# cics-nd/gptorch

Measured on AMD Instinct MI355X. Metric: GP log-marginal-likelihood evals/sec (Cholesky+solve) at NxD fp64, higher is better.
Workload: dtype f64; 1 GPU; C3: GPR+Matern52 N=32768 D=16 fp64 LML eval; N=32768, D=16, dy=1, kernel=Matern52, parallelism=1 GPU

## Files before the change

### gptorch_amd/_native.py

```python
import ctypes
import os

_HERE = os.path.dirname(os.path.abspath(__file__))
LIB_PATH = os.environ.get("GPN_LIB", os.path.join(_HERE, "lib", "libgpnative.so"))

c_void_p, c_int, c_int64, c_double = ctypes.c_void_p, ctypes.c_int, ctypes.c_int64, ctypes.c_double

SIGNATURES = {
    "gpn_version": (c_int, []),
    "gpn_arch": (ctypes.c_char_p, []),
    "gpn_last_hip_error": (ctypes.c_char_p, []),
    "gpn_factor_ld": (c_int64, [c_int64, c_int64]),
    "gpn_factor_rows": (c_int64, [c_int64, c_int64]),
    "gpn_winv_bytes": (c_int64, [c_int64]),
    "gpn_kernel_matrix": (c_int, [c_void_p, c_int, c_void_p, c_int64, c_void_p, c_int64, c_int,
                                  c_void_p, c_void_p, c_int, c_void_p, c_int, c_void_p, c_int64]),
    "gpn_pack_rhs": (c_int, [c_void_p, c_void_p, c_void_p, c_int64, c_int, c_void_p, c_int64]),
    "gpn_potrf_lower": (c_int, [c_void_p, c_void_p, c_int64, c_int64, c_int64, c_void_p, c_void_p]),
    "gpn_potrf_lower_panel": (c_int, [c_void_p, c_void_p, c_int64, c_int64, c_int64, c_void_p, c_void_p]),
    "gpn_potrf_lower_batched": (c_int, [c_void_p, c_void_p, c_int64, c_int64, c_int64, c_int64, c_void_p, c_int64, c_void_p, c_int]),
    "gpn_lml_reduce_batched": (c_int, [c_void_p, c_void_p, c_int64, c_int64, c_int64, c_int64, c_void_p, c_int]),
    "gpn_lml_forward_batched": (c_int, [c_void_p, c_int, c_int, c_void_p, c_int64, c_int64, c_int, c_void_p, c_int64, c_void_p, c_int64, c_int,
                                        c_void_p, c_void_p, c_int, c_void_p, c_void_p, c_int64, c_int64, c_void_p, c_int64, c_void_p, c_void_p]),
    "gpn_potrf_panel_width": (c_int64, [c_int64]),
    "gpn_potrf_panel_levels": (c_int, [c_int64, c_void_p]),
    "gpn_potrf_lower_persistent": (c_int, [c_void_p, c_void_p, c_int64, c_int64, c_int64, c_void_p, c_void_p]),
    "gpn_potrf_persistent_supported": (c_int, [c_int64, c_int64]),
    "gpn_potrf_persistent_plan": (c_int, [c_int64, c_int64, c_void_p, c_void_p, c_int64, c_void_p, c_int64]),
    "gpn_release_stream": (c_int, [c_void_p]),
    "gpn_trtri_diag": (c_int, [c_void_p, c_void_p, c_int64, c_int64, c_void_p, c_void_p]),
    "gpn_trsm_right_lt": (c_int, [c_void_p, c_void_p, c_int64, c_int64, c_void_p, c_void_p, c_int64, c_int64]),
    "gpn_lml_reduce": (c_int, [c_void_p, c_void_p, c_int64, c_int64, c_int64, c_void_p]),
    "gpn_gemm_nt": (c_int, [c_void_p, c_int64, c_int64, c_int64, c_double, c_void_p, c_int64,
                            c_void_p, c_int64, c_double, c_void_p, c_int64, c_int, c_int]),
    "gpn_gemm_nt_stair": (c_int, [c_void_p, c_int64, c_int64, c_int64, c_int64, c_double, c_void_p, c_int64,
                                  c_void_p, c_int64, c_double, c_void_p, c_int64, c_int64, c_int]),
    "gpn_gemm_nt_batched": (c_int, [c_void_p, c_int64, c_int64, c_int64, c_double, c_void_p, c_int64, c_int64,
                                    c_void_p, c_int64, c_int64, c_double, c_void_p, c_int64, c_int64, c_int, c_int, c_int]),
    "gpn_gemm_nt_batched_scaled": (c_int, [c_void_p, c_int64, c_int64, c_int64, c_void_p, c_void_p, c_int64, c_int64,
                                           c_void_p, c_int64, c_int64, c_double, c_void_p, c_int64, c_int64, c_int, c_int, c_int]),
    "gpn_kernel_matrix_batched": (c_int, [c_void_p, c_int, c_int, c_void_p, c_int64, c_int64, c_void_p, c_int64, c_int64, c_int,
                                          c_void_p, c_void_p, c_int, c_void_p, c_int, c_void_p, c_int64, c_int64]),
    "gpn_trsm_right_lt_batched": (c_int, [c_void_p, c_void_p, c_int64, c_int64, c_int64, c_void_p, c_int64,
                                          c_void_p, c_int64, c_int64, c_int64, c_int]),
    "gpn_trtri_upper_batched": (c_int, [c_void_p, c_void_p, c_int64, c_int64, c_int64, c_void_p, c_int64,
                                        c_void_p, c_int64, c_int64, c_void_p, c_int64, c_int64, c_int]),
    "gpn_kernel_grad_batched": (c_int, [c_void_p, c_int, c_int, c_void_p, c_int64, c_int64, c_void_p, c_int64, c_int64, c_int,
                                        c_void_p, c_void_p, c_int, c_void_p, c_int64, c_int64, c_void_p, c_void_p]),
    "gpn_kernel_grad_x2_batched": (c_int, [c_void_p, c_int, c_int, c_void_p, c_int64, c_int64, c_void_p, c_int64, c_int64, c_int,
                                           c_void_p, c_void_p, c_int, c_void_p, c_int64, c_int64, c_double, c_int, c_void_p, c_void_p]),
    "gpn_dot2d_batched": (c_int, [c_void_p, c_void_p, c_int64, c_int64, c_void_p, c_int64, c_int64, c_int64, c_int64, c_void_p, c_int]),
    "gpn_lml_forward_ragged": (c_int, [c_void_p, c_int, c_int, c_void_p, c_int64, c_int64, c_void_p, c_int, c_void_p, c_int64, c_int,
                                       c_void_p, c_void_p, c_int, c_void_p, c_void_p, c_int64, c_int64, c_void_p, c_int64, c_void_p, c_void_p]),
    "gpn_lml_backward_ragged": (c_int, [c_void_p, c_int, c_int, c_void_p, c_int64, c_int64, c_void_p, c_int, c_void_p, c_void_p, c_int,
                                        c_void_p, c_int64, c_int64, c_void_p, c_int64, c_int, c_void_p, c_void_p]),
    "gpn_trtri_upper": (c_int, [c_void_p, c_void_p, c_int64, c_int64, c_void_p, c_void_p, c_int64]),
    "gpn_trtri_upper_ws": (c_int, [c_void_p, c_void_p, c_int64, c_int64, c_void_p, c_void_p, c_int64, c_void_p, c_int64]),
    "gpn_grad_work_bytes": (c_int64, [c_int64, c_int64, c_int, c_int]),
    "gpn_lml_grad": (c_int, [c_void_p, c_int, c_void_p, c_int64, c_int, c_void_p, c_void_p, c_int,
                             c_void_p, c_int64, c_void_p, c_int64, c_int, c_void_p, c_void_p]),
    "gpn_kernel_grad": (c_int, [c_void_p, c_int, c_void_p, c_int64, c_void_p, c_int64, c_int, c_void_p, c_void_p,
                                c_int, c_void_p, c_int64, c_void_p, c_void_p]),
    "gpn_grad_x2_work_bytes": (c_int64, [c_int64, c_int64, c_int]),
    "gpn_kernel_grad_x2": (c_int, [c_void_p, c_int, c_void_p, c_int64, c_void_p, c_int64, c_int, c_void_p, c_void_p,
                                   c_int, c_void_p, c_int64, c_double, c_int, c_void_p, c_void_p]),
    "gpn_lml_forward": (c_int, [c_void_p, c_int, c_void_p, c_int64, c_int, c_void_p, c_void_p, c_int, c_void_p, c_void_p,
                                c_int, c_void_p, c_void_p, c_int64, c_void_p, c_void_p, c_void_p]),
    "gpn_lml_forward_saving": (c_int, [c_void_p, c_int, c_void_p, c_int64, c_int, c_void_p, c_void_p, c_int, c_void_p, c_void_p,
                                       c_int, c_void_p, c_void_p, c_int64, c_void_p, c_void_p, c_void_p, c_void_p]),
    "gpn_lml_refine_work_bytes": (c_int64, [c_int64, c_int]),
    "gpn_lml_refine": (c_int, [c_void_p, c_int, c_void_p, c_int64, c_int, c_void_p, c_void_p, c_int, c_void_p, c_void_p,
                               c_int, c_void_p, c_void_p, c_int64, c_void_p, c_void_p, c_void_p]),
    "gpn_lml_backward_work_bytes": (c_int64, [c_int64, c_int, c_int]),
    "gpn_lml_backward": (c_int, [c_void_p, c_int, c_void_p, c_int64, c_int, c_void_p, c_void_p, c_int,
                                 c_void_p, c_int64, c_void_p, c_int, c_void_p, c_void_p, c_void_p]),
    "gpn_lml_backward_batched_work_bytes": (c_int64, [c_int64, c_int, c_int, c_int]),
    "gpn_lml_backward_batched": (c_int, [c_void_p, c_int, c_int, c_void_p, c_int64, c_int64, c_int, c_void_p, c_void_p, c_int,
                                         c_void_p, c_int64, c_int64, c_void_p, c_int64, c_int, c_void_p, c_void_p, c_void_p]),
    "gpn_lml_kinv_layout": (c_int, [c_int64, c_int, ctypes.POINTER(c_int64)]),
    "gpn_lml_kinv_batched_work_bytes": (c_int64, [c_int64, c_int, c_int]),
    "gpn_lml_kinv_batched": (c_int, [c_void_p, c_int, c_int64, c_void_p, c_int64, c_int64, c_void_p, c_int64, c_int, c_void_p]),
    "gpn_lml_grad_batched": (c_int, [c_void_p, c_int, c_int, c_void_p, c_int64, c_int64, c_int, c_void_p, c_void_p, c_int,
                                     c_void_p, c_int64, c_int64, c_void_p, c_int64, c_int64, c_int, c_void_p, c_void_p]),
    "gpn_predict_work_bytes": (c_int64, [c_int64, c_int64, c_int]),
    "gpn_predict": (c_int, [c_void_p, c_int, c_void_p, c_int64, c_int, c_void_p, c_int64, c_void_p, c_void_p, c_void_p, c_int,
                            c_void_p, c_int64, c_void_p, c_int, c_int, c_void_p, c_void_p, c_void_p]),
    "gpn_block_inverse_bytes": (c_int64, [c_int64]),
    "gpn_block_inverse": (c_int, [c_void_p, c_void_p, c_int64, c_int64, c_void_p, c_void_p]),
    "gpn_trsm_right_lt_blocked": (c_int, [c_void_p, c_void_p, c_int64, c_int64, c_void_p, c_void_p, c_int64, c_int64, c_void_p, c_int64]),
    "gpn_predict_blocked": (c_int, [c_void_p, c_int, c_void_p, c_int64, c_int, c_void_p, c_int64, c_void_p, c_void_p, c_void_p, c_int,
                                    c_void_p, c_int64, c_void_p, c_void_p, c_int, c_int, c_void_p, c_void_p, c_void_p]),
    "gpn_transpose": (c_int, [c_void_p, c_void_p, c_int64, c_int64, c_int64, c_void_p, c_int64]),
    "gpn_copy_matrix": (c_int, [c_void_p, c_void_p, c_int64, c_int64, c_int64, c_void_p, c_int64, c_int]),
    "gpn_row_sumsq": (c_int, [c_void_p, c_void_p, c_int64, c_int64, c_int64, c_void_p]),
    "gpn_fill_zero": (c_int, [c_void_p, c_void_p, c_int64]),
    "gpn_gemv_t_work_bytes": (c_int64, [c_int64, c_int64, c_int]),
    "gpn_gemv_t_acc": (c_int, [c_void_p, c_void_p, c_int64, c_int64, c_int64, c_void_p, c_int64, c_int, c_void_p, c_int64, c_void_p]),
    "gpn_refine_tile_count": (c_int64, [c_int64]),
    "gpn_refine_resid_part_work_bytes": (c_int64, [c_int, c_int64]),
    "gpn_refine_resid_part": (c_int, [c_void_p, c_int, c_void_p, c_int64, c_int, c_void_p, c_void_p, c_int, c_void_p,
                                      c_void_p, c_int, c_int64, c_int64, c_void_p, c_void_p]),
    "gpn_svgp_marginals": (c_int, [c_void_p, c_void_p, c_int64, c_void_p, c_int64, c_int64, c_int64, c_void_p, c_int64, c_int,
                                   c_void_p, c_int64, c_void_p, c_void_p]),
    "gpn_svgp_backward_rows": (c_int, [c_void_p, c_void_p, c_int64, c_void_p, c_int64, c_int64, c_int64, c_void_p, c_int64, c_int,
                                       c_void_p, c_void_p, c_void_p, c_void_p, c_int64]),
    "gpn_refine_finish": (c_int, [c_void_p, c_void_p, c_void_p, c_void_p, c_void_p, c_int64, c_int, c_void_p]),
}
class ExprTerm(ctypes.Structure):
    _fields_ = [("type", c_int), ("kind", c_int), ("var_off", c_int), ("ls_off", c_int), ("nls", c_int), ("nvar", c_int)]


TERM_STATIONARY, TERM_LINEAR, TERM_CONSTANT, TERM_WHITE = 0, 1, 2, 3
EXPR_MAX_TERMS, EXPR_MAX_GROUPS = 16, 8
SIGNATURES.update({
    "gpn_lml_refine_dense": (c_int, [c_void_p, c_void_p, c_int64, c_double, c_int64, c_void_p, c_void_p, c_int, c_void_p, c_int64, c_void_p, c_void_p, c_void_p]),
    "gpn_lml_refine_expr": (c_int, [c_void_p, ctypes.POINTER(ExprTerm), c_int, ctypes.POINTER(c_int), c_int, c_void_p, c_void_p, c_int64, c_int,
                                    c_void_p, c_void_p, c_int, c_void_p, c_void_p, c_int64, c_void_p, c_void_p, c_void_p]),
    "gpn_refine_resid_part_expr": (c_int, [c_void_p, ctypes.POINTER(ExprTerm), c_int, ctypes.POINTER(c_int), c_int, c_void_p, c_void_p, c_int64, c_int,
                                           c_void_p, c_void_p, c_int, c_int64, c_int64, c_void_p, c_void_p]),
    "gpn_kernel_matrix_expr": (c_int, [c_void_p, ctypes.POINTER(ExprTerm), c_int, ctypes.POINTER(c_int), c_int, c_void_p, c_void_p,
                                       c_int64, c_void_p, c_int64, c_int, c_void_p, c_int, c_void_p, c_int64]),
    "gpn_kernel_expr_grad_work_bytes": (c_int64, [c_int64, c_int64, c_int, c_int]),
    "gpn_kernel_matrix_expr_batched": (c_int, [c_void_p, ctypes.POINTER(ExprTerm), c_int, ctypes.POINTER(c_int), c_int, c_int, c_void_p,
                                               c_int64, c_void_p, c_int64, c_int64, c_int, c_void_p, c_void_p, c_int64, c_int64]),
    "gpn_kernel_expr_grad_batched": (c_int, [c_void_p, ctypes.POINTER(ExprTerm), c_int, ctypes.POINTER(c_int), c_int, c_int, c_void_p,
                                             c_int64, c_int, c_void_p, c_int64, c_int64, c_int, c_void_p, c_int64, c_int64, c_void_p,
                                             c_int64, c_int64, c_int, c_int, c_void_p, c_void_p]),
    "gpn_kernel_expr_grad": (c_int, [c_void_p, ctypes.POINTER(ExprTerm), c_int, ctypes.POINTER(c_int), c_int, c_void_p, c_int,
                                     c_void_p, c_int64, c_void_p, c_int64, c_int, c_void_p, c_int64, c_void_p, c_int64, c_int, c_int,
                                     c_void_p, c_void_p]),
})

BCAST_FN = ctypes.CFUNCTYPE(c_int, c_void_p, c_int, c_void_p, c_int64, c_int, c_void_p)
ALLREDUCE_FN = ctypes.CFUNCTYPE(c_int, c_void_p, c_void_p, c_int64, c_void_p)


class DistComm(ctypes.Structure):
    _fields_ = [("ctx", c_void_p), ("bcast", BCAST_FN), ("allreduce", ALLREDUCE_FN), ("flags", c_int)]


SIGNATURES.update({
    "gpn_dist_work_bytes": (c_int64, [c_int, c_int, c_int, c_int64, c_int, c_int, c_int64]),
    "gpn_dist_lml_refine_work_bytes": (c_int64, [c_int, c_int, c_int, c_int64, c_int, c_int, c_int64]),
    "gpn_dist_grad_work_bytes": (c_int64, [c_int, c_int, c_int, c_int64, c_int, c_int, c_int64]),
    "gpn_dist_lml_grad": (c_int, [c_void_p, ctypes.POINTER(DistComm), c_int, c_int, c_int, c_int, c_void_p, c_int64, c_int,
                                  c_void_p, c_int, c_void_p, c_void_p, c_int, c_void_p, c_int64, c_void_p, c_int64, c_void_p,
                                  c_void_p, c_void_p]),
    "gpn_dist_layout": (c_int, [c_int, c_int, c_int, c_int, c_int64, c_int, c_int, c_int64, ctypes.POINTER(c_int64), c_int]),
    "gpn_dist_predict_work_bytes": (c_int64, [c_int, c_int, c_int, c_int64, c_int, c_int, c_int64, c_int64, c_int]),
    "gpn_dist_predict": (c_int, [c_void_p, ctypes.POINTER(DistComm), c_int, c_int, c_int, c_int, c_void_p, c_int64, c_int,
                                 c_void_p, c_int, c_void_p, c_int64, c_void_p, c_void_p, c_void_p, c_int, c_void_p, c_int64, c_int,
                                 c_void_p, c_int64, c_void_p, c_void_p, c_void_p]),
    "gpn_dist_lml_forward": (c_int, [c_void_p, ctypes.POINTER(DistComm), c_int, c_int, c_int, c_int, c_void_p, c_int64, c_int,
                                     c_void_p, c_int, c_void_p, c_void_p, c_int, c_void_p, c_int64, c_void_p, c_int64, c_void_p]),
    "gpn_dist_lml_refine": (c_int, [c_void_p, ctypes.POINTER(DistComm), c_int, c_int, c_int, c_int, c_void_p, c_int64, c_int,
                                    c_void_p, c_int, c_void_p, c_void_p, c_int, c_void_p, c_int64, c_void_p, c_void_p, c_int64, c_void_p]),
})
RCCL_LIB_PATH = os.environ.get("GPN_RCCL_LIB", os.path.join(os.path.dirname(LIB_PATH), "libgpnative_rccl.so"))
RCCL_SIGNATURES = {
    "gpn_rccl_comm_create": (ctypes.POINTER(DistComm), [c_void_p, c_void_p, c_void_p]),
    "gpn_rccl_comm_destroy": (None, [ctypes.POINTER(DistComm)]),
    "gpn_mesh_plan": (c_int64, [c_int, c_int, c_int, c_int64, c_int, c_int64, ctypes.POINTER(c_int64), c_int64]),
}
DIST_FORCE_COLLECTIVES, DIST_MESH_EXCHANGE = 1, 2
_rccl_lib = None


def rccl_lib():
    global _rccl_lib
    if _rccl_lib is None:
        if not os.path.exists(RCCL_LIB_PATH):
            raise NativeError("libgpnative_rccl.so not found at %s -- run gptorch_amd/csrc/build.sh" % RCCL_LIB_PATH)
        handle = ctypes.CDLL(RCCL_LIB_PATH)
        for name, (res, args) in RCCL_SIGNATURES.items():
            fn = getattr(handle, name)
            fn.restype, fn.argtypes = res, args
        _rccl_lib = handle
    return _rccl_lib


PROFILE_SIGNATURES = {
    "gpn_profile_enable": (c_int, [c_int]),
    "gpn_profile_collect": (c_int, [ctypes.POINTER(c_double)]),
    "gpn_profile_collect_classes": (c_int, [ctypes.POINTER(c_double), c_int]),
}
SIGNATURES.update(PROFILE_SIGNATURES)
DEBUG_SIGNATURES = {
    "gpn_debug_set_gemm_variant": (c_int, [c_int]),
    "gpn_debug_set_potrf_variant": (c_int, [c_int]),
    "gpn_debug_set_outer_width": (c_int, [c_int, c_int]),
    "gpn_debug_set_extra_rows": (c_int, [c_int]),
    "gpn_debug_set_thin_tiles": (c_int, [c_int]),
    "gpn_debug_masked_stream": (c_int, [ctypes.POINTER(ctypes.c_uint32), c_int, ctypes.POINTER(c_void_p)]),
    "gpn_debug_set_backsub_persistent": (c_int, [c_int]),
    "gpn_debug_set_persistent": (c_int, [c_int, c_int]),
    "gpn_debug_persistent_trace": (c_int, [c_void_p]),
}
DEBUG_LIB_PATH = os.path.join(_HERE, "lib", "libgpnative_dbg.so")

_lib = None
_product_lib = None
_debug_lib = None


class NativeError(RuntimeError):
    pass


def _load(path, extra):
    handle = ctypes.CDLL(path)
    for name, (res, args) in list(SIGNATURES.items()) + list(extra.items()):
        fn = getattr(handle, name)
        fn.restype, fn.argtypes = res, args
    return handle


def lib():
    global _lib, _product_lib
    if _lib is None:
        if not os.path.exists(LIB_PATH):
            raise NativeError(
                "libgpnative.so not found at %s -- build it with `python -c 'import __graft_entry__ as g; "
                "g.build()'` (or gptorch_amd/csrc/build.sh). gptorch_amd has no CPU fallback." % LIB_PATH)
        extra = DEBUG_SIGNATURES if os.path.basename(LIB_PATH).startswith("libgpnative_dbg") else {}
        _product_lib = _lib = _load(LIB_PATH, extra)
    return _lib


class debug_library:

    def __enter__(self):
        global _lib, _debug_lib
        lib()
        if _debug_lib is None:
            if not os.path.exists(DEBUG_LIB_PATH):
                raise NativeError("libgpnative_dbg.so not found at %s -- run gptorch_amd/csrc/build.sh" % DEBUG_LIB_PATH)
            _debug_lib = _load(DEBUG_LIB_PATH, DEBUG_SIGNATURES)
        _lib = _debug_lib
        return _debug_lib

    def __exit__(self, *exc):
        global _lib
        _debug_lib.gpn_debug_set_gemm_variant(0)
        _debug_lib.gpn_debug_set_potrf_variant(0)
        _lib = _product_lib
        return False


_debug_ctx = None


def debug_begin():
    global _debug_ctx
    if _debug_ctx is None:
        _debug_ctx = debug_library()
        return _debug_ctx.__enter__()
    return _debug_lib


def debug_end():
    global _debug_ctx
    if _debug_ctx is not None:
        _debug_ctx.__exit__(None, None, None)
        _debug_ctx = None


def check(status, what):
    if status != 0:
        detail = lib().gpn_last_hip_error().decode() if status == -100 else ""
        raise NativeError("%s failed with status %d %s" % (what, status, detail))
```

### gptorch_amd/csrc/gemm_f64.hip

```cpp
#include <algorithm>
#include <atomic>
#include <type_traits>
#include <cstdlib>
#include "gpn_common.h"
#include "gemm_tile.h"

namespace gpn {

template <int BM, int BN, int WM, int WN, bool DMA, int NS = 2, bool BLOW = false, bool PIPE = false>
__global__ __launch_bounds__(64 * (BM / WM) * (BN / WN), ((BM / WM) * (BN / WN) > 8 ? 1 : 2)) void gemm_nt_kernel(GemmArgs p) {
  gemm_nt_tile<BM, BN, WM, WN, DMA, NS, BLOW, PIPE>(p, (int)blockIdx.x, (int)gridDim.x, false);
}

GPN_SWITCH int g_gemm_variant = 0;
GPN_SWITCH int g_thin_tiles = 1;
GPN_SWITCH int g_smem_pad = 0;
static constexpr int g_group_h = 8;
static constexpr int g_big_tile_min_trapezoid = 4096;

static int64_t stair_tiles(int64_t M, int64_t N, int st_blk, int st_step, int st_diag, int64_t b) {
  const int64_t mt = (M + b - 1) / b, bt = st_blk / b, nb = N / st_blk, stept = st_step / b;
  int64_t total = 0;
  for (int64_t k = 0; k < nb; ++k) {
    const int64_t rows_t = std::max<int64_t>(mt - k * stept, 0);
    total += rows_t * bt - ((st_diag && rows_t >= bt) ? bt * (bt - 1) / 2 : 0);
  }
  return total;
}

template <int BM, int BN, int WM, int WN, bool DMA, int NS = 2, bool BLOW = false, bool PIPE = false>
static int launch(hipStream_t s, const GemmArgs& a0, int inplace = 0) {
  GemmArgs a = a0;
  a.mt = (a.M + BM - 1) / BM;
  a.nt = (a.N + BN - 1) / BN;
  if (a.lower == 3 && (BM != BN || a.st_blk % BN || a.st_step % BM)) return GPN_E_UNSUPPORTED;
  const int grid = (a.lower == 3   ? (int)stair_tiles(a.M, a.N, a.st_blk, a.st_step, a.st_diag, BM)
                    : a.lower == 2 ? (a.mt - a.nt) * a.nt + a.nt * (a.nt + 1) / 2
                    : a.lower      ? a.mt * (a.mt + 1) / 2 : a.mt * a.nt) * std::max(1, a.batch);
  if (grid <= 0) return GPN_OK;
  const int smem = ((BM + BN) / 16) * 2 * 1024 * NS + g_smem_pad * 1024;
  auto kern = gemm_nt_kernel<BM, BN, WM, WN, DMA, NS, BLOW, PIPE>;
  static std::atomic<int> attr_set{-1};
  if (attr_set.load(std::memory_order_acquire) < smem) {
    GPN_HIP_CHECK(hipFuncSetAttribute(reinterpret_cast<const void*>(kern),
                                      hipFuncAttributeMaxDynamicSharedMemorySize, smem));
    attr_set.store(smem, std::memory_order_release);
  }
  const bool prof = profile_on();
  int rec = -1;
  if (prof) {
    const double tiles = (a.lower == 3   ? (double)stair_tiles(a.M, a.N, a.st_blk, a.st_step, a.st_diag, BM)
                          : a.lower == 2 ? (double)(a.mt - a.nt) * a.nt + 0.5 * a.nt * (a.nt + 1.0)
                          : a.lower      ? 0.5 * a.mt * (a.mt + 1.0) : (double)a.mt * a.nt) * std::max(1, a.batch);
    const int cls = inplace ? PROF_GEMM_SOLVE : (a.tri ? PROF_GEMM_TRI : (a.lower == 1 ? PROF_GEMM_SYRK : PROF_GEMM));
    rec = profile_begin(s, tiles * 2.0 * BM * BN * (double)a.K, cls);
  }
  hipLaunchKernelGGL(kern, dim3(grid), dim3(64 * (BM / WM) * (BN / WN)), smem, s, a);
  if (prof) profile_end(s, rec);
  GPN_LAUNCH_CHECK();
  return GPN_OK;
}

struct Stair { int blk = 0, step = 0, diag = 0; };
struct Outer { int count = 0; int64_t sA = 0, sB = 0, sC = 0; };
static int gemm_nt_impl(hipStream_t s, int64_t M, int64_t N, int64_t K, double alpha,
                        const double* A, int64_t lda, const double* B, int64_t ldb,
                        double beta, double* C, int64_t ldc, int lower, int tri, int inplace,
                        int batch, int64_t sA, int64_t sB, int64_t sC, Stair st = Stair(), Outer ob = Outer(),
                        const double* alpha_dev = nullptr);

int gemm_nt(hipStream_t s, int64_t M, int64_t N, int64_t K, double alpha,
            const double* A, int64_t lda, const double* B, int64_t ldb,
            double beta, double* C, int64_t ldc, int lower, int tri, int inplace) {
  return gemm_nt_impl(s, M, N, K, alpha, A, lda, B, ldb, beta, C, ldc, lower, tri, inplace, 1, 0, 0, 0);
}

int gemm_nt_batched(hipStream_t s, int64_t M, int64_t N, int64_t K, double alpha,
                    const double* A, int64_t lda, int64_t sA, const double* B, int64_t ldb, int64_t sB,
                    double beta, double* C, int64_t ldc, int64_t sC, int tri, int batch) {
  return gemm_nt_impl(s, M, N, K, alpha, A, lda, B, ldb, beta, C, ldc, 0, tri, 0, batch, sA, sB, sC);
}

int gemm_nt_strided(hipStream_t s, int64_t M, int64_t N, int64_t K, double alpha,
                    const double* A, int64_t lda, const double* B, int64_t ldb,
                    double beta, double* C, int64_t ldc, int lower, int tri, int inplace,
                    int batch, int64_t sA, int64_t sB, int64_t sC) {
  return gemm_nt_impl(s, M, N, K, alpha, A, lda, B, ldb, beta, C, ldc, lower, tri, inplace, batch, sA, sB, sC);
}

int gemm_nt_strided2(hipStream_t s, int64_t M, int64_t N, int64_t K, double alpha,
                     const double* A, int64_t lda, const double* B, int64_t ldb,
                     double beta, double* C, int64_t ldc, int lower, int tri,
                     int inner, int64_t sA, int64_t sB, int64_t sC, int outer, int64_t sA2, int64_t sB2, int64_t sC2) {
  if (inner <= 1) return gemm_nt_impl(s, M, N, K, alpha, A, lda, B, ldb, beta, C, ldc, lower, tri, 0, outer, sA2, sB2, sC2);
  if (outer <= 1) return gemm_nt_impl(s, M, N, K, alpha, A, lda, B, ldb, beta, C, ldc, lower, tri, 0, inner, sA, sB, sC);
  Outer ob;
  ob.count = outer; ob.sA = sA2; ob.sB = sB2; ob.sC = sC2;
  return gemm_nt_impl(s, M, N, K, alpha, A, lda, B, ldb, beta, C, ldc, lower, tri, 0, inner, sA, sB, sC, Stair(), ob);
}

int gemm_nt_stair(hipStream_t s, int64_t M, int64_t nblocks, int64_t blk, int64_t K, double alpha,
                  const double* A, int64_t lda, const double* B, int64_t ldb,
                  double beta, double* C, int64_t ldc, int64_t step, int diag) {
  Stair st;
  st.blk = (int)blk; st.step = (int)step; st.diag = diag ? 1 : 0;
  return gemm_nt_impl(s, M, nblocks * blk, K, alpha, A, lda, B, ldb, beta, C, ldc, 3, 0, 0, 1, 0, 0, 0, st);
}

static int gemm_nt_impl(hipStream_t s, int64_t M, int64_t N, int64_t K, double alpha,
                        const double* A, int64_t lda, const double* B, int64_t ldb,
                        double beta, double* C, int64_t ldc, int lower, int tri, int inplace,
                        int batch, int64_t sA, int64_t sB, int64_t sC, Stair st, Outer ob, const double* alpha_dev) {
  if (M <= 0 || N <= 0 || batch <= 0) return GPN_OK;
  GemmArgs a;
  a.alpha_dev = alpha_dev;
  a.batch = batch; a.sA = sA; a.sB = sB; a.sC = sC;
  a.inner = 0; a.sA2 = a.sB2 = a.sC2 = 0;
  a.acc_in = nullptr; a.acc_out = nullptr;
  if (ob.count > 0) {
    a.inner = batch; a.sA2 = ob.sA; a.sB2 = ob.sB; a.sC2 = ob.sC;
    a.batch = batch = batch * ob.count;
  }
  a.A = A; a.B = B; a.C = C;
  a.lda = lda; a.ldb = ldb; a.ldc = ldc;
  a.M = (int)M; a.N = (int)N; a.K = (int)K;
  a.mt = a.nt = 0;
  a.lower = lower;
  a.st_blk = st.blk; a.st_step = st.step; a.st_diag = st.diag;
  a.group_h = g_group_h;
  a.thin = g_thin_tiles;
  a.tri = tri;
  a.alpha = alpha; a.beta = beta;
  auto tiles = [&](int64_t b) {
    const int64_t mt = (M + b - 1) / b, nt = (N + b - 1) / b;
    if (lower == 3) return stair_tiles(M, N, st.blk, st.step, st.diag, b);
    return (lower == 2 ? (mt - nt) * nt + nt * (nt + 1) / 2 : lower ? mt * (mt + 1) / 2 : mt * nt) * batch;
  };
  const int64_t t128 = tiles(128), t64 = tiles(64);
  const bool small = tri ? !(K >= 8192 && t128 >= (lower ? 4096 : 8192) && M > 64 && N > 64)
                         : !(K >= 512 && t128 >= (lower == 2 ? g_big_tile_min_trapezoid : 4096) && M > 64 && N > 64);
  if (inplace) {
    if (N > 128 || K > 128 || lower) return GPN_E_UNSUPPORTED;
    if (g_gemm_variant == 2) return launch<64, 128, 32, 64, true>(s, a, 1);
    return (tri & GPN_TRI_B_LOWER) ? launch<32, 128, 16, 64, true, 4, true>(s, a, 1) : launch<32, 128, 16, 64, true, 4>(s, a, 1);
  }
  if (g_gemm_variant == 3) return launch<128, 128, 64, 64, true>(s, a);
  if (g_gemm_variant == 4) return launch<64, 64, 32, 32, true>(s, a);
  if (g_gemm_variant == 5) return launch<64, 64, 32, 32, true, 8>(s, a);
  if (g_gemm_variant == 6) return launch<32, 32, 16, 16, true, 8>(s, a);
  if (g_gemm_variant == 7) return launch<128, 128, 64, 64, true, 2, false, true>(s, a);
  if (g_gemm_variant == 8) return launch<64, 64, 32, 32, true, 2, false, true>(s, a);
  if (g_gemm_variant == 9) return launch<128, 128, 64, 32, true, 2, false, true>(s, a);
  if (g_gemm_variant == 10) return launch<128, 128, 64, 32, true, 2, false, false>(s, a);
  if (g_gemm_variant == 11) return launch<128, 128, 32, 64, true, 2, false, true>(s, a);
  const bool std_path = g_gemm_variant == 0 || g_gemm_variant == 21;
  if (std_path && (M <= 32 || N <= 32)) return launch<32, 32, 16, 16, true, 8>(s, a);
  if (std_path && (t64 <= 64 || (N <= 128 && t64 <= 128))) {
    return launch<32, 32, 16, 16, true, 8>(s, a);
  }
  if (std_path) {
    if (small) return launch<64, 64, 32, 32, true, 2, false, true>(s, a);
    if (g_gemm_variant == 21) return launch<128, 128, 64, 64, true, 2, false, true>(s, a);
    return launch<128, 128, 32, 64, true, 2, false, true>(s, a);
  }
  return small ? launch<64, 64, 32, 32, false>(s, a) : launch<128, 128, 64, 64, false>(s, a);
}

}

extern "C" int gpn_gemm_nt_stair(void* stream, int64_t M, int64_t nblocks, int64_t blk, int64_t K, double alpha,
                                 const double* A, int64_t lda, const double* B, int64_t ldb,
                                 double beta, double* C, int64_t ldc, int64_t step, int diag) {
  if (M < 0) return -2;
  if (nblocks < 0) return -3;
  if (blk <= 0 || (blk % 128)) return -4;
  if (K <= 0 || (K % 16)) return -5;
  if (step < 0 || (step % 128)) return -14;
  if (diag && M < blk) return -15;
  if (diag)
    for (int64_t b = 1; b < nblocks; ++b) {
      const int64_t rows = M - b * step;
      if (rows > 0 && rows < blk) return -15;
    }
  if ((lda & 1) || (ldb & 1)) return GPN_E_ALIGN;
  if ((reinterpret_cast<uintptr_t>(A) & 15) || (reinterpret_cast<uintptr_t>(B) & 15)) return GPN_E_ALIGN;
  if (M == 0 || nblocks == 0) return GPN_OK;
  return gpn::gemm_nt_stair(static_cast<hipStream_t>(stream), M, nblocks, blk, K, alpha, A, lda, B, ldb, beta, C, ldc, step, diag);
}

GPN_DEBUG_ONLY(
extern "C" int gpn_debug_set_thin_tiles(int on) { gpn::g_thin_tiles = on; return GPN_OK; }
extern "C" int gpn_debug_set_gemm_variant(int v) {
  gpn::g_gemm_variant = v & 0x7f;
  gpn::g_smem_pad = v >> 8;
  return GPN_OK;
})

extern "C" int gpn_gemm_nt_batched(void* stream, int64_t M, int64_t N, int64_t K, double alpha,
                                   const double* A, int64_t lda, int64_t sA, const double* B, int64_t ldb, int64_t sB,
                                   double beta, double* C, int64_t ldc, int64_t sC, int lower, int tri, int batch) {
  if (M < 0) return -2;
  if (N < 0) return -3;
  if (K < 0 || (K % 16) != 0) return -4;
  if (batch < 1) return -18;
  if (M == 0 || N == 0) return GPN_OK;
  if (!A) return -6;
  if (!B) return -9;
  if (!C) return -13;
  if (lower && M != N) return -16;
  if ((lda % 2) || (ldb % 2) || (sA % 2) || (sB % 2)) return GPN_E_ALIGN;
  if ((reinterpret_cast<uintptr_t>(A) & 15) || (reinterpret_cast<uintptr_t>(B) & 15)) return GPN_E_ALIGN;
  return gpn::gemm_nt_impl(static_cast<hipStream_t>(stream), M, N, K, alpha, A, lda, B, ldb, beta, C, ldc,
                           lower ? 1 : 0, tri, 0, batch, sA, sB, sC);
}

extern "C" int gpn_gemm_nt_batched_scaled(void* stream, int64_t M, int64_t N, int64_t K, const double* alphas,
                                          const double* A, int64_t lda, int64_t sA, const double* B, int64_t ldb, int64_t sB,
                                          double beta, double* C, int64_t ldc, int64_t sC, int lower, int tri, int batch) {
  if (M < 0) return -2;
  if (N < 0) return -3;
  if (K <= 0 || (K % 16) != 0) return -4;
  if (!alphas) return -5;
  if (batch < 1) return -18;
  if (M == 0 || N == 0) return GPN_OK;
  if (!A) return -6;
  if (!B) return -9;
  if (!C) return -13;
  if (lower && M != N) return -16;
  if (tri < 0 || tri > 15) return -17;
  if ((lda % 2) || (ldb % 2) || (sA % 2) || (sB % 2)) return GPN_E_ALIGN;
  if ((reinterpret_cast<uintptr_t>(A) & 15) || (reinterpret_cast<uintptr_t>(B) & 15)) return GPN_E_ALIGN;
  return gpn::gemm_nt_impl(static_cast<hipStream_t>(stream), M, N, K, 0.0, A, lda, B, ldb, beta, C, ldc,
                           lower ? 1 : 0, tri, 0, batch, sA, sB, sC, gpn::Stair(), gpn::Outer(), alphas);
}

extern "C" int gpn_gemm_nt(void* stream, int64_t M, int64_t N, int64_t K, double alpha,
                           const double* A, int64_t lda, const double* B, int64_t ldb,
                           double beta, double* C, int64_t ldc, int lower, int tri) {
  if (M < 0) return -2;
  if (N < 0) return -3;
  if (K < 0 || (K % 16) != 0) return -4;
  if (lower < 0 || lower > 2) return -13;
  if (lower == 1 && M != N) return -13;
  if (lower == 2 && (M < N || tri)) return -13;
  if ((lda & 1) || (ldb & 1)) return GPN_E_ALIGN;
  if ((reinterpret_cast<uintptr_t>(A) & 15) || (reinterpret_cast<uintptr_t>(B) & 15)) return GPN_E_ALIGN;
  if (K == 0) {
    return GPN_E_UNSUPPORTED;
  }
  if (tri < 0 || tri > 15) return -14;
  return gpn::gemm_nt(static_cast<hipStream_t>(stream), M, N, K, alpha, A, lda, B, ldb, beta, C, ldc, lower, tri, 0);
}
```

### gptorch_amd/csrc/gemm_tile.h

```cpp
#pragma once
#include <type_traits>
#include "gpn_common.h"

namespace gpn {

typedef double d4 __attribute__((ext_vector_type(4)));
typedef double d2 __attribute__((ext_vector_type(2)));

struct GemmArgs {
  const double* A;
  const double* B;
  double* C;
  int64_t lda, ldb, ldc;
  int M, N, K;
  int mt, nt;
  int lower;
  int group_h;
  int thin;
  int st_blk, st_step, st_diag;
  int tri;
  double alpha, beta;
  int batch;
  int64_t sA, sB, sC;
  int inner;
  int64_t sA2, sB2, sC2;
  const double* acc_in;
  double* acc_out;
  const double* alpha_dev = nullptr;
};

__device__ __forceinline__ int xcd_remap(int bid, int nwg) {
  const int xcd = bid & 7, q = nwg >> 3, r = nwg & 7;
  return (xcd < r ? xcd * (q + 1) : r * (q + 1) + (xcd - r) * q) + (bid >> 3);
}

__device__ __forceinline__ void tile_of_block(int bid, int nwg, int mt, int nt, bool spread, int& ti, int& tj, int GH = 8) {
  const int logical = spread ? bid : xcd_remap(bid, nwg);
  const int group = GH * nt;
  const int g = logical / group;
  const int first = g * GH;
  const int gm = min(GH, mt - first);
  const int rem = logical - g * group;
  ti = first + rem % gm;
  tj = rem / gm;
}

__device__ __forceinline__ void lower_tile_of_index(int q, int mt, int& ti, int& tj, int GH = 8);
__device__ __forceinline__ void tile_of_block_lower(int bid, int nwg, int mt, bool spread, int& ti, int& tj, int GH = 8) {
  lower_tile_of_index(spread ? bid : xcd_remap(bid, nwg), mt, ti, tj, GH);
}
__device__ __forceinline__ void lower_tile_of_index(int q, int mt, int& ti, int& tj, int GH) {
  const int G = mt / GH;
  const int tri = GH * (GH + 1) / 2, sq = GH * GH;
  auto before = [&](int g) { return sq * (g * (g - 1) / 2) + g * tri; };
  const int full_total = before(G);
  int g, h;
  if (q < full_total) {
    const double a = 0.5 * sq, b = (double)tri - 0.5 * sq;
    g = (int)((sqrt(b * b + 4.0 * a * (double)q) - b) / (2.0 * a));
    while (g > 0 && before(g) > q) --g;
    while (before(g + 1) <= q) ++g;
    h = GH;
  } else {
    g = G;
    h = mt - G * GH;
  }
  int r = q - before(g);
  const int left = h * GH * g;
  if (r < left) {
    tj = r / h;
    ti = GH * g + r - tj * h;
  } else {
    r -= left;
    int c = 0;
    while (r >= h - c) { r -= h - c; ++c; }
    ti = GH * g + c + r;
    tj = GH * g + c;
  }
}

template <int BM, int BN, int WM, int WN, bool DMA, int NS = 2, bool BLOW = false, bool PIPE = false, bool XW = false, bool WT = false>
__device__ __forceinline__ void gemm_nt_tile(GemmArgs p, int bid, int nwg, const bool direct, const int tid_in = -1) {
  constexpr int TM = WM / 16, TN = WN / 16;
  constexpr int WAVES_N = BN / WN;
  constexpr int BK = 16;
  constexpr int A_BLOCKS = (BM / 16) * 2, B_BLOCKS = (BN / 16) * 2;
  constexpr int NBLK = A_BLOCKS + B_BLOCKS;
  constexpr int NWAVES = (BM / WM) * (BN / WN);
  constexpr int PER_WAVE = (NBLK + NWAVES - 1) / NWAVES;
  constexpr int STAGE = NBLK * 1024;
  extern __shared__ __attribute__((aligned(16))) char smem[];

  int ti, tj;
  const bool spread = direct || (p.tri & (GPN_TRI_A_UPPER | GPN_TRI_A_LOWER | GPN_TRI_B_UPPER)) != 0;
  if (p.batch > 1) {
    nwg = nwg / p.batch;
    const int z = bid / nwg;
    bid -= z * nwg;
    if (p.inner > 0) {
      const int z2 = z / p.inner, z1 = z - z2 * p.inner;
      p.A += z1 * p.sA + z2 * p.sA2; p.B += z1 * p.sB + z2 * p.sB2; p.C += z1 * p.sC + z2 * p.sC2;
    } else {
      p.A += z * p.sA; p.B += z * p.sB; p.C += z * p.sC;
    }
    if (p.alpha_dev) p.alpha = p.alpha_dev[z];
  } else if (p.alpha_dev) {
    p.alpha = p.alpha_dev[0];
  }
  int diag_off = 0;
  bool stair_diag_tile = false;
  if (p.lower == 3) {
    int q = xcd_remap(bid, nwg);
    const int bt = p.st_blk / BN, nb = p.nt / bt, stept = p.st_step / BM;
    int b = 0, sbt = 0, rows_t = 0, cnt = 0;
    for (; b < nb; ++b) {
      sbt = b * stept;
      rows_t = max(p.mt - sbt, 0);
      cnt = rows_t * bt - ((p.st_diag && rows_t >= bt) ? bt * (bt - 1) / 2 : 0);
      if (q < cnt) break;
      q -= cnt;
    }
    if (p.st_diag && rows_t >= bt) {
      const int rect = (rows_t - bt) * bt;
      if (q < rect) {
        tile_of_block(q, rect, rows_t - bt, bt, true, ti, tj, p.group_h);
        ti += sbt + bt;
      } else {
        tile_of_block_lower(q - rect, bt * (bt + 1) / 2, bt, true, ti, tj, p.group_h);
        stair_diag_tile = ti == tj;
        ti += sbt;
      }
    } else {
      tile_of_block(q, cnt, rows_t, bt, true, ti, tj, p.group_h);
      ti += sbt;
    }
    tj += b * bt;
    diag_off = sbt * BM - b * bt * BN;
  } else if (p.lower == 2) {
    const int rect = (p.mt - p.nt) * p.nt;
    const int q = xcd_remap(bid, nwg);
    if (q < rect) {
      tile_of_block(q, rect, p.mt - p.nt, p.nt, true, ti, tj, p.group_h);
      ti += p.nt;
    } else {
      tile_of_block_lower(q - rect, nwg - rect, p.nt, true, ti, tj, p.group_h);
    }
  } else if (p.lower) tile_of_block_lower(bid, nwg, p.mt, spread, ti, tj, p.group_h);
  else tile_of_block(bid, nwg, p.mt, p.nt, spread, ti, tj, p.group_h);

  const int tid = tid_in >= 0 ? tid_in : (int)threadIdx.x;
  const int lane = tid & 63;
  const int wave = __builtin_amdgcn_readfirstlane(tid >> 6);
  const int wave_m = wave / WAVES_N, wave_n = wave % WAVES_N;
  const int m0 = ti * BM, n0 = tj * BN;
  const int mlim = (p.M + 15) & ~15, nlim = (p.N + 15) & ~15;

  const int R16 = lane & 15;
  const int roff0 = (R16 >> 3) * 1024 + ((R16 & 7) * 8 + ((lane >> 4) ^ ((R16 >> 1) & 7))) * 16;

  d4 acc[TM][TN];
#pragma unroll
  for (int i = 0; i < TM; ++i)
#pragma unroll
    for (int j = 0; j < TN; ++j) acc[i][j] = d4{0.0, 0.0, 0.0, 0.0};

  d2 stage_regs[DMA ? 1 : PER_WAVE];

  const double* src_base[PER_WAVE];
  bool src_ok[PER_WAVE];
#pragma unroll
  for (int i = 0; i < PER_WAVE; ++i) {
    const int idx = wave + NWAVES * i;
    const bool isA = idx < A_BLOCKS;
    const int b = isA ? idx : idx - A_BLOCKS;
    const int rg = b >> 1, half = b & 1;
    const int row = (isA ? m0 : n0) + rg * 16;
    src_ok[i] = (idx < NBLK) && row < (isA ? mlim : nlim);
    const int srow = src_ok[i] ? row : 0;
    const int r16 = half * 8 + (lane >> 3);
    const int seg = (lane & 7) ^ ((r16 >> 1) & 7);
    src_base[i] = (isA ? p.A + (int64_t)(srow + r16) * p.lda : p.B + (int64_t)(srow + r16) * p.ldb) + seg * 2;
  }

  auto stage_issue = [&](int t, int s) {
    const int k0 = t * BK;
#pragma unroll
    for (int i = 0; i < PER_WAVE; ++i) {
      const int idx = wave + NWAVES * i;
      const double* src = src_base[i] + k0;
      if constexpr (DMA) {
        if (NBLK % NWAVES == 0 || idx < NBLK) {
          char* dst = smem + s * STAGE + idx * 1024;
          __builtin_amdgcn_global_load_lds(
              (const __attribute__((address_space(1))) void*)src,
              (__attribute__((address_space(3))) void*)dst, 16, 0, 0);
        }
      } else {
        stage_regs[i] = src_ok[i] ? *reinterpret_cast<const d2*>(src) : d2{0.0, 0.0};
      }
    }
  };
  auto stage_issue_piece = [&](int i, int t, int s) {
    if constexpr (DMA) {
      const int idx = wave + NWAVES * i;
      char* dst = smem + s * STAGE + idx * 1024;
      __builtin_amdgcn_global_load_lds(
          (const __attribute__((address_space(1))) void*)(src_base[i] + t * BK),
          (__attribute__((address_space(3))) void*)dst, 16, 0, 0);
    }
  };
  auto stage_commit = [&](int s) {
    if constexpr (!DMA) {
#pragma unroll
      for (int i = 0; i < PER_WAVE; ++i) {
        const int idx = wave + NWAVES * i;
        if (idx < NBLK) *reinterpret_cast<d2*>(smem + s * STAGE + idx * 1024 + lane * 16) = stage_regs[i];
      }
    }
  };

  auto compute = [&](int s, int k0) {
    const char* base = smem + s * STAGE;
#pragma unroll
    for (int kg8 = 0; kg8 < 2; ++kg8) {
      d2 a[TM], b[TN];
#pragma unroll
      for (int i = 0; i < TM; ++i)
        a[i] = *reinterpret_cast<const d2*>(base + (wave_m * TM + i) * 2048 + (kg8 ? (roff0 ^ 64) : roff0));
#pragma unroll
      for (int j = 0; j < TN; ++j)
        b[j] = *reinterpret_cast<const d2*>(base + (A_BLOCKS + (wave_n * TN + j) * 2) * 1024 + (kg8 ? (roff0 ^ 64) : roff0));
      if constexpr (BLOW) {
#pragma unroll
        for (int j = 0; j < TN; ++j) {
          if (k0 + kg8 * 8 > n0 + wave_n * WN + j * 16 + 15) continue;
#pragma unroll
          for (int i = 0; i < TM; ++i) {
            acc[i][j] = __builtin_amdgcn_mfma_f64_16x16x4f64(a[i].x, b[j].x, acc[i][j], 0, 0, 0);
            acc[i][j] = __builtin_amdgcn_mfma_f64_16x16x4f64(a[i].y, b[j].y, acc[i][j], 0, 0, 0);
          }
        }
      } else {
#pragma unroll
        for (int i = 0; i < TM; ++i)
#pragma unroll
          for (int j = 0; j < TN; ++j) {
            acc[i][j] = __builtin_amdgcn_mfma_f64_16x16x4f64(a[i].x, b[j].x, acc[i][j], 0, 0, 0);
            acc[i][j] = __builtin_amdgcn_mfma_f64_16x16x4f64(a[i].y, b[j].y, acc[i][j], 0, 0, 0);
          }
      }
    }
  };

  int k_lo = 0, k_hi = p.K;
  if (p.tri & GPN_TRI_A_UPPER) k_lo = max(k_lo, m0);
  if (p.tri & GPN_TRI_B_UPPER) k_lo = max(k_lo, n0);
  if (p.tri & GPN_TRI_A_LOWER) k_hi = min(k_hi, m0 + BM);
  if (p.tri & GPN_TRI_B_LOWER) k_hi = min(k_hi, n0 + BN);
  const int t0 = k_lo / BK;
  const int nk = max(t0, (k_hi + BK - 1) / BK);
  if constexpr (XW) {
    static_assert(NS == 2 && PIPE, "extra waves: the pipelined two-stage loop only");
    if (wave >= NWAVES) {
      const bool thin_x = p.thin && (p.M - m0) <= 16 && p.lower != 3;
      if (thin_x) {
        for (int t = t0; t < nk; ++t) __syncthreads();
      } else if (t0 < nk) {
        __syncthreads();
        for (int t = t0; t < nk; ++t) __syncthreads();
      }
      return;
    }
  }
  if constexpr (NS == 2) {
    if constexpr (PIPE) {
      static_assert(DMA && !BLOW && PER_WAVE % TM == 0, "pipelined loop: LDS-DMA staging, whole pieces per MFMA group");
      d2 a0[TM], b0[TN], a1[TM], b1[TN];
      auto read_ops = [&](int s, int kg8, d2 (&a)[TM], d2 (&b)[TN]) {
        const char* base = smem + s * STAGE;
#pragma unroll
        for (int i = 0; i < TM; ++i)
          a[i] = *reinterpret_cast<const d2*>(base + (wave_m * TM + i) * 2048 + (kg8 ? (roff0 ^ 64) : roff0));
#pragma unroll
        for (int j = 0; j < TN; ++j)
          b[j] = *reinterpret_cast<const d2*>(base + (A_BLOCKS + (wave_n * TN + j) * 2) * 1024 + (kg8 ? (roff0 ^ 64) : roff0));
      };
      auto mfma_groups = [&](d2 (&a)[TM], d2 (&b)[TN], int i_lo, int i_hi, auto issue_c, int tnext, int snext) {
        constexpr bool issue = decltype(issue_c)::value;
        constexpr int PG = PER_WAVE / TM;
#pragma unroll
        for (int i = 0; i < TM; ++i) {
          if (i < i_lo || i >= i_hi) continue;
#pragma unroll
          for (int j = 0; j < TN; ++j) {
            acc[i][j] = __builtin_amdgcn_mfma_f64_16x16x4f64(a[i].x, b[j].x, acc[i][j], 0, 0, 0);
            acc[i][j] = __builtin_amdgcn_mfma_f64_16x16x4f64(a[i].y, b[j].y, acc[i][j], 0, 0, 0);
          }
          if constexpr (issue) {
#pragma unroll
            for (int q = 0; q < PG; ++q) stage_issue_piece(i * PG + q, tnext, snext);
            __builtin_amdgcn_sched_barrier(0);
          }
        }
      };
      auto kstep = [&](int t, auto issue_c, bool read_next) {
        const int s = t & 1;
        mfma_groups(a0, b0, 0, 1, std::false_type{}, 0, 0);
        __builtin_amdgcn_sched_barrier(0);
        read_ops(s, 1, a1, b1);
        __builtin_amdgcn_sched_barrier(0);
        mfma_groups(a0, b0, 1, TM, std::false_type{}, 0, 0);
        __builtin_amdgcn_sched_barrier(0);
        __syncthreads();
        mfma_groups(a1, b1, 0, 1, issue_c, t + 2, s);
        __builtin_amdgcn_sched_barrier(0);
        if (read_next) read_ops(s ^ 1, 0, a0, b0);
        __builtin_amdgcn_sched_barrier(0);
        mfma_groups(a1, b1, 1, TM, issue_c, t + 2, s);
        __builtin_amdgcn_sched_barrier(0);
      };
      const bool thin = p.thin && (p.M - m0) <= 16 && p.lower != 3;
      if (thin) {
        if (t0 < nk) stage_issue(t0, t0 & 1);
        for (int t = t0; t < nk; ++t) {
          const int s = t & 1;
          __syncthreads();
          if (t + 1 < nk) stage_issue(t + 1, s ^ 1);
          if (wave_m == 0) {
            const char* base = smem + s * STAGE;
#pragma unroll
            for (int kg8 = 0; kg8 < 2; ++kg8) {
              const d2 av = *reinterpret_cast<const d2*>(base + (kg8 ? (roff0 ^ 64) : roff0));
#pragma unroll
              for (int j = 0; j < TN; ++j) {
                const d2 bv = *reinterpret_cast<const d2*>(base + (A_BLOCKS + (wave_n * TN + j) * 2) * 1024 + (kg8 ? (roff0 ^ 64) : roff0));
                acc[0][j] = __builtin_amdgcn_mfma_f64_16x16x4f64(av.x, bv.x, acc[0][j], 0, 0, 0);
                acc[0][j] = __builtin_amdgcn_mfma_f64_16x16x4f64(av.y, bv.y, acc[0][j], 0, 0, 0);
              }
            }
          }
          __builtin_amdgcn_sched_barrier(0);
        }
      } else if (t0 < nk) {
        stage_issue(t0, t0 & 1);
        if constexpr (WT) {
          if (p.acc_in) {
            const double* ai = p.acc_in + (int64_t)wave * (TM * TN * 4 * 64) + lane;
#pragma unroll
            for (int i = 0; i < TM; ++i)
#pragma unroll
              for (int j = 0; j < TN; ++j)
#pragma unroll
                for (int r = 0; r < 4; ++r) acc[i][j][r] = ai[((i * TN + j) * 4 + r) * 64];
          }
        }
        __syncthreads();
        read_ops(t0 & 1, 0, a0, b0);
        if (t0 + 1 < nk) stage_issue(t0 + 1, (t0 + 1) & 1);
        int t = t0;
        for (; t + 2 < nk; ++t) kstep(t, std::true_type{}, true);
        for (; t < nk; ++t) kstep(t, std::false_type{}, t + 1 < nk);
      }
    } else {
      if (t0 < nk) {
        stage_issue(t0, t0 & 1);
        stage_commit(t0 & 1);
      }
      for (int t = t0; t < nk; ++t) {
        const int s = t & 1;
        __syncthreads();
        if (t + 1 < nk) stage_issue(t + 1, s ^ 1);
        compute(s, t * BK);
        __builtin_amdgcn_sched_barrier(0);
        if (t + 1 < nk) stage_commit(s ^ 1);
      }
    }
  } else {
    static_assert(DMA, "the ring is LDS-DMA only");
    static_assert(NBLK % NWAVES == 0, "equal DMA count per wave");
    constexpr int AHEAD = NS - 1;
    for (int t = t0; t < min(nk, t0 + AHEAD); ++t) stage_issue(t, (t - t0) % NS);
    for (int t = t0; t < nk; ++t) {
      const int slot = (t - t0) % NS;
      if (t + AHEAD <= nk) {
        asm volatile("s_waitcnt vmcnt(%0)" ::"n"(PER_WAVE * (AHEAD - 1)) : "memory");
      } else {
        asm volatile("s_waitcnt vmcnt(0)" ::: "memory");
      }
      __builtin_amdgcn_s_barrier();
      if (t + AHEAD < nk) stage_issue(t + AHEAD, (t - t0 + AHEAD) % NS);
      compute(slot, t * BK);
      __builtin_amdgcn_sched_barrier(0);
    }
  }

  const int crow = lane >> 4, ccol = lane & 15;
  const bool diag_tile = p.lower == 3 ? stair_diag_tile : (p.lower && (ti == tj));
  const bool use_c = p.beta != 0.0;
  if constexpr (WT) {
    if (p.acc_out) {
#pragma unroll
      for (int i = 0; i < TM; ++i)
#pragma unroll
        for (int j = 0; j < TN; ++j)
#pragma unroll
          for (int r = 0; r < 4; ++r)
            __hip_atomic_store(&p.acc_out[((((int64_t)wave * TM + i) * TN + j) * 4 + r) * 64 + lane], acc[i][j][r], __ATOMIC_RELAXED,
                               __HIP_MEMORY_SCOPE_AGENT);
      return;
    }
  }
#pragma unroll
  for (int i = 0; i < TM; ++i) {
    double cold[TN][4];
    bool ok[TN][4];
#pragma unroll
    for (int j = 0; j < TN; ++j) {
      const int col = n0 + wave_n * WN + j * 16 + ccol;
#pragma unroll
      for (int r = 0; r < 4; ++r) {
        const int row = m0 + wave_m * WM + i * 16 + crow + 4 * r;
        ok[j][r] = row < p.M && col < p.N && (!diag_tile || col + diag_off <= row);
        cold[j][r] = 0.0;
        if (use_c && ok[j][r]) cold[j][r] = p.C[(int64_t)row * p.ldc + col];
      }
    }
#pragma unroll
    for (int j = 0; j < TN; ++j) {
      const int col = n0 + wave_n * WN + j * 16 + ccol;
#pragma unroll
      for (int r = 0; r < 4; ++r) {
        const int row = m0 + wave_m * WM + i * 16 + crow + 4 * r;
        if (ok[j][r]) {
          const double v = fma(p.beta, cold[j][r], p.alpha * acc[i][j][r]);
          if constexpr (WT) __hip_atomic_store(&p.C[(int64_t)row * p.ldc + col], v, __ATOMIC_RELAXED, __HIP_MEMORY_SCOPE_AGENT);
          else p.C[(int64_t)row * p.ldc + col] = v;
        }
      }
    }
  }
}

}
```

Before: 5.400 LML evals/s.

## Issue second GEMM stage early and prefetch C during final k-step

In the pipelined fp64 GEMM tile loop, the prologue now issues the second LDS-DMA stage before the first barrier and waits on a counted vmcnt, so the two stage loads overlap. On the last k-step, full interior tiles with nonzero beta prefetch their C rows while the MFMAs are still running, and the epilogue then writes C directly from the prefetched values. Occupancy hints for small pipelined tiles are also raised. The cost is extra registers for the C prefetch, plus added reliance on hand-written waitcnt and barrier ordering, which could break correctness or occupancy if the counts are wrong.

```diff
diff --git a/gptorch_amd/_native.py b/gptorch_amd/_native.py
--- a/gptorch_amd/_native.py
+++ b/gptorch_amd/_native.py
@@ -191,6 +191,7 @@
     "gpn_debug_set_outer_width": (c_int, [c_int, c_int]),
     "gpn_debug_set_extra_rows": (c_int, [c_int]),
     "gpn_debug_set_thin_tiles": (c_int, [c_int]),
+    "gpn_debug_set_gemm_opt": (c_int, [c_int]),
     "gpn_debug_masked_stream": (c_int, [ctypes.POINTER(ctypes.c_uint32), c_int, ctypes.POINTER(c_void_p)]),
     "gpn_debug_set_backsub_persistent": (c_int, [c_int]),
     "gpn_debug_set_persistent": (c_int, [c_int, c_int]),
@@ -242,6 +243,7 @@
     def __exit__(self, *exc):
         global _lib
         _debug_lib.gpn_debug_set_gemm_variant(0)
+        _debug_lib.gpn_debug_set_gemm_opt(-1)
         _debug_lib.gpn_debug_set_potrf_variant(0)
         _lib = _product_lib
         return False
diff --git a/gptorch_amd/csrc/gemm_f64.hip b/gptorch_amd/csrc/gemm_f64.hip
--- a/gptorch_amd/csrc/gemm_f64.hip
+++ b/gptorch_amd/csrc/gemm_f64.hip
@@ -8,13 +8,14 @@
 namespace gpn {
 
 template <int BM, int BN, int WM, int WN, bool DMA, int NS = 2, bool BLOW = false, bool PIPE = false>
-__global__ __launch_bounds__(64 * (BM / WM) * (BN / WN), ((BM / WM) * (BN / WN) > 8 ? 1 : 2)) void gemm_nt_kernel(GemmArgs p) {
+__global__ __launch_bounds__(64 * (BM / WM) * (BN / WN), ((BM / WM) * (BN / WN) > 8 ? 1 : (PIPE && BM * BN <= 4096) ? 5 : 2)) void gemm_nt_kernel(GemmArgs p) {
   gemm_nt_tile<BM, BN, WM, WN, DMA, NS, BLOW, PIPE>(p, (int)blockIdx.x, (int)gridDim.x, false);
 }
 
 GPN_SWITCH int g_gemm_variant = 0;
 GPN_SWITCH int g_thin_tiles = 1;
 GPN_SWITCH int g_smem_pad = 0;
+GPN_SWITCH int g_gemm_opt = GEMM_OPT_SHIPPED;
 static constexpr int g_group_h = 8;
 static constexpr int g_big_tile_min_trapezoid = 4096;
 
@@ -129,6 +130,7 @@
   a.st_blk = st.blk; a.st_step = st.step; a.st_diag = st.diag;
   a.group_h = g_group_h;
   a.thin = g_thin_tiles;
+  a.opt = g_gemm_opt;
   a.tri = tri;
   a.alpha = alpha; a.beta = beta;
   auto tiles = [&](int64_t b) {
@@ -190,6 +192,7 @@
 
 GPN_DEBUG_ONLY(
 extern "C" int gpn_debug_set_thin_tiles(int on) { gpn::g_thin_tiles = on; return GPN_OK; }
+extern "C" int gpn_debug_set_gemm_opt(int bits) { gpn::g_gemm_opt = bits < 0 ? gpn::GEMM_OPT_SHIPPED : bits; return GPN_OK; }
 extern "C" int gpn_debug_set_gemm_variant(int v) {
   gpn::g_gemm_variant = v & 0x7f;
   gpn::g_smem_pad = v >> 8;
diff --git a/gptorch_amd/csrc/gemm_tile.h b/gptorch_amd/csrc/gemm_tile.h
--- a/gptorch_amd/csrc/gemm_tile.h
+++ b/gptorch_amd/csrc/gemm_tile.h
@@ -6,6 +6,9 @@
 
 typedef double d4 __attribute__((ext_vector_type(4)));
 typedef double d2 __attribute__((ext_vector_type(2)));
+
+enum : int { GEMM_OPT_EARLY_STAGE = 1, GEMM_OPT_C_PREFETCH = 2 };
+constexpr int GEMM_OPT_SHIPPED = GEMM_OPT_EARLY_STAGE | GEMM_OPT_C_PREFETCH;
 
 struct GemmArgs {
   const double* A;
@@ -27,6 +30,7 @@
   const double* acc_in;
   double* acc_out;
   const double* alpha_dev = nullptr;
+  int opt = GEMM_OPT_SHIPPED;
 };
 
 __device__ __forceinline__ int xcd_remap(int bid, int nwg) {
@@ -166,6 +170,35 @@
 
   d2 stage_regs[DMA ? 1 : PER_WAVE];
 
+  constexpr bool CPRE = PIPE && !WT && TM * TN <= 4;
+  typedef __attribute__((address_space(1))) char gchar;
+  typedef __attribute__((address_space(1))) double gdouble;
+  double cpre[CPRE ? TM : 1][CPRE ? TN : 1][4];
+  unsigned c_lane = 0;
+  gchar* c_wave = nullptr;
+  auto c_begin = [&]() {
+    c_lane = ((unsigned)(lane >> 4) * (unsigned)p.ldc + (unsigned)(lane & 15)) * 8u;
+    const uint64_t u = reinterpret_cast<uint64_t>(p.C + (int64_t)(m0 + wave_m * WM) * p.ldc + (n0 + wave_n * WN));
+    const unsigned hi = (unsigned)__builtin_amdgcn_readfirstlane((int)(u >> 32)), lo = (unsigned)__builtin_amdgcn_readfirstlane((int)u);
+    c_wave = reinterpret_cast<gchar*>(((uint64_t)hi << 32) | (uint64_t)lo);
+  };
+  auto c_elem = [&](int i, int j, int r) -> gdouble* {
+    return reinterpret_cast<gdouble*>(c_wave + ((int64_t)(i * 16 + 4 * r) * p.ldc + j * 16) * 8 + c_lane);
+  };
+  auto c_load_rows = [&](int i_lo, int i_hi) {
+    if constexpr (CPRE) {
+#pragma unroll
+      for (int i = 0; i < TM; ++i) {
+        if (i < i_lo || i >= i_hi) continue;
+#pragma unroll
+        for (int j = 0; j < TN; ++j)
+#pragma unroll
+          for (int r = 0; r < 4; ++r) cpre[i][j][r] = *c_elem(i, j, r);
+      }
+    }
+  };
+  auto c_prefetch = [&]() { c_load_rows(0, 1); };
+
   const double* src_base[PER_WAVE];
   bool src_ok[PER_WAVE];
 #pragma unroll
@@ -259,6 +292,19 @@
   if (p.tri & GPN_TRI_B_LOWER) k_hi = min(k_hi, n0 + BN);
   const int t0 = k_lo / BK;
   const int nk = max(t0, (k_hi + BK - 1) / BK);
+  auto c_finish = [&](bool diag_tile) {
+    c_load_rows(1, TM);
+    const int crow = lane >> 4, ccol = lane & 15;
+#pragma unroll
+    for (int i = 0; i < TM; ++i)
+#pragma unroll
+      for (int j = 0; j < TN; ++j)
+#pragma unroll
+        for (int r = 0; r < 4; ++r) {
+          const int row = m0 + wave_m * WM + i * 16 + crow + 4 * r, col = n0 + wave_n * WN + j * 16 + ccol;
+          if (!diag_tile || col + diag_off <= row) *c_elem(i, j, r) = fma(p.beta, cpre[i][j][r], p.alpha * acc[i][j][r]);
+        }
+  };
   if constexpr (XW) {
     static_assert(NS == 2 && PIPE, "extra waves: the pipelined two-stage loop only");
     if (wave >= NWAVES) {
@@ -275,7 +321,9 @@
   if constexpr (NS == 2) {
     if constexpr (PIPE) {
       static_assert(DMA && !BLOW && PER_WAVE % TM == 0, "pipelined loop: LDS-DMA staging, whole pieces per MFMA group");
+      static_assert(NBLK % NWAVES == 0, "equal DMA count per wave (the counted wait of the prologue)");
       d2 a0[TM], b0[TN], a1[TM], b1[TN];
+      bool c_early = false;
       auto read_ops = [&](int s, int kg8, d2 (&a)[TM], d2 (&b)[TN]) {
         const char* base = smem + s * STAGE;
 #pragma unroll
@@ -303,7 +351,8 @@
           }
         }
       };
-      auto kstep = [&](int t, auto issue_c, bool read_next) {
+      auto kstep = [&](int t, auto issue_c, bool read_next, auto c_now_c) {
+        constexpr bool c_now = decltype(c_now_c)::value;
         const int s = t & 1;
         mfma_groups(a0, b0, 0, 1, std::false_type{}, 0, 0);
         __builtin_amdgcn_sched_barrier(0);
@@ -311,7 +360,17 @@
         __builtin_amdgcn_sched_barrier(0);
         mfma_groups(a0, b0, 1, TM, std::false_type{}, 0, 0);
         __builtin_amdgcn_sched_barrier(0);
-        __syncthreads();
+        if constexpr (c_now) {
+          if (c_early) {
+            c_prefetch();
+            __builtin_amdgcn_sched_barrier(0);
+            __builtin_amdgcn_s_barrier();
+          } else {
+            __syncthreads();
+          }
+        } else {
+          __syncthreads();
+        }
         mfma_groups(a1, b1, 0, 1, issue_c, t + 2, s);
         __builtin_amdgcn_sched_barrier(0);
         if (read_next) read_ops(s ^ 1, 0, a0, b0);
@@ -354,12 +413,34 @@
                 for (int r = 0; r < 4; ++r) acc[i][j][r] = ai[((i * TN + j) * 4 + r) * 64];
           }
         }
-        __syncthreads();
-        read_ops(t0 & 1, 0, a0, b0);
-        if (t0 + 1 < nk) stage_issue(t0 + 1, (t0 + 1) & 1);
+        if (p.opt & GEMM_OPT_EARLY_STAGE) {
+          const bool two = t0 + 1 < nk;
+          if (two) stage_issue(t0 + 1, (t0 + 1) & 1);
+          bool counted = two;
+          if constexpr (WT) counted = counted && !p.acc_in;
+          if (counted) asm volatile("s_waitcnt vmcnt(%0)" ::"n"(PER_WAVE) : "memory");
+          else asm volatile("s_waitcnt vmcnt(0)" ::: "memory");
+          __builtin_amdgcn_s_barrier();
+          read_ops(t0 & 1, 0, a0, b0);
+        } else {
+          __syncthreads();
+          read_ops(t0 & 1, 0, a0, b0);
+          if (t0 + 1 < nk) stage_issue(t0 + 1, (t0 + 1) & 1);
+        }
         int t = t0;
-        for (; t + 2 < nk; ++t) kstep(t, std::true_type{}, true);
-        for (; t < nk; ++t) kstep(t, std::false_type{}, t + 1 < nk);
+        for (; t + 2 < nk; ++t) kstep(t, std::true_type{}, true, std::false_type{});
+        if constexpr (CPRE)
+          c_early = (p.opt & GEMM_OPT_C_PREFETCH) && p.beta != 0.0 && p.ldc < (1 << 26) && m0 + (wave_m + 1) * WM <= p.M && n0 + (wave_n + 1) * WN <= p.N;
+        if (t + 2 == nk) {
+          kstep(t, std::false_type{}, true, std::false_type{});
+          ++t;
+        }
+        if (c_early) c_begin();
+        kstep(t, std::false_type{}, false, std::true_type{});
+        if (c_early) {
+          c_finish(p.lower == 3 ? stair_diag_tile : (p.lower && (ti == tj)));
+          return;
+        }
       }
     } else {
       if (t0 < nk) {
```

Result: no change. 5.444 LML evals/s (median of 6 runs) (+0.8%).
